# facebookresearch/pytorch3d

Hardware: AMD Instinct MI355X
Metric: rasterized Mpix/s (fwd+bwd) at 512^2 faces_per_pixel=8 (higher is better)
Workload: dtype f32

## Files before the change

pytorch3d_amd/csrc/p3d_geom.h:

```cpp
#pragma once

#include <math.h>
#include <stdint.h>

#if defined(__HIPCC__)
#define P3D_HD __host__ __device__ __forceinline__
#define P3D_HDM __host__ __device__ __forceinline__
#else
#define P3D_HD static inline
#define P3D_HDM inline
#endif

namespace p3d {

#define P3D_KEPS 1e-8

struct f2 {
  float x, y;
};
struct f3 {
  float x, y, z;
};

P3D_HD f2 mk2(float x, float y) {
// ... 179 lines not shown
  f3 v0, v1, v2;
  double rd_area;
  double rd_l01, rd_l02, rd_l12;
  bool wide;
  f2 d01, d12, d20;
};

P3D_HD float edge_fn_d(f2 p, f2 a, f2 d) { return (p.x - a.x) * d.y - (p.y - a.y) * d.x; }

P3D_HD double edge_recip(f2 a, f2 b) {
  const float bax = b.x - a.x;
  const float bay = b.y - a.y;
  const float l2 = bax * bax + bay * bay;
  return ((double)l2 <= P3D_KEPS) ? -1.0 : recip_for_div_wide(l2);
}

P3D_HD void face_rec_make(f3 v0, f3 v1, f3 v2, FaceRec* r) {
  const f2 a = mk2(v0.x, v0.y), b = mk2(v1.x, v1.y), c = mk2(v2.x, v2.y);
  const float area = bary_area(a, b, c);
  r->v0 = v0;
  r->v1 = v1;
  r->v2 = v2;
  r->rd_area = recip_for_div_wide(area);
  r->rd_l01 = edge_recip(a, b);
  r->rd_l02 = edge_recip(a, c);
  r->rd_l12 = edge_recip(b, c);
  r->d01 = mk2(b.x - a.x, b.y - a.y);
  r->d12 = mk2(c.x - b.x, c.y - b.y);
  r->d20 = mk2(a.x - c.x, a.y - c.y);
  const float big = fmaxf(fmaxf(fmaxf(fabsf(v0.x), fabsf(v0.y)), fmaxf(fabsf(v1.x), fabsf(v1.y))),
                          fmaxf(fmaxf(fabsf(v2.x), fabsf(v2.y)), max3(fabsf(v0.z), fabsf(v1.z), fabsf(v2.z))));
  r->wide = !((big <= 1024.0f) & (fabsf(area) >= 1e-9f));
}

template <bool PROPER = false>
P3D_HD float seg_dist2_rec(f2 p, f2 a, f2 b, f2 ba, double rd_l2) {
  const float bax = ba.x;
  const float bay = ba.y;
  float t = exact_div(bax * (p.x - a.x) + bay * (p.y - a.y), rd_l2);
  t = sat01(t);
  const float dx = (a.x + t * bax) - p.x;
  const float dy = (a.y + t * bay) - p.y;
  const float d_seg = dx * dx + dy * dy;
  if (PROPER) return d_seg;
  const float ex = p.x - b.x;
  const float ey = p.y - b.y;
  const float d_point = ex * ex + ey * ey;
  return (rd_l2 < 0.0) ? d_point : d_seg;
}

P3D_HD bool face_rec_degenerate(const FaceRec& r) { return (r.rd_l01 < 0.0) | (r.rd_l02 < 0.0) | (r.rd_l12 < 0.0); }

P3D_HD f3 face_depth_rec(const FaceRec& r, f2 p, bool perspective_correct, bool clip_bary, FaceHit* out) {
  const f2 a = mk2(r.v0.x, r.v0.y);
  const f2 b = mk2(r.v1.x, r.v1.y);
  const f2 c = mk2(r.v2.x, r.v2.y);
  const f3 bw = mk3(exact_div(edge_fn_d(p, b, r.d12), r.rd_area), exact_div(edge_fn_d(p, c, r.d20), r.rd_area),
                    exact_div(edge_fn_d(p, a, r.d01), r.rd_area));
  f3 bp = bw;
  if (perspective_correct) {
    const float t0 = bw.x * r.v1.z * r.v2.z;
    const float t1 = r.v0.z * bw.y * r.v2.z;
    const float t2 = r.v0.z * r.v1.z * bw.z;
    const float denom = fmaxf(t0 + t1 + t2, (float)P3D_KEPS);
    const double rd = r.wide ? recip_for_div_wide(denom) : recip_for_div(denom);
    bp = mk3(exact_div(t0, rd), exact_div(t1, rd), exact_div(t2, rd));
  }
  f3 bc = bp;
  if (clip_bary) {
    const float w0 = bp.x > 0.0f ? bp.x : 0.0f;
    const float w1 = bp.y > 0.0f ? bp.y : 0.0f;
    const float w2 = bp.z > 0.0f ? bp.z : 0.0f;
    float s = w0 + w1 + w2;
    s = fmaxf(s, 1e-5f);
    const double rd = r.wide ? recip_for_div_wide(s) : recip_for_div(s);
    bc = mk3(exact_div(w0, rd), exact_div(w1, rd), exact_div(w2, rd));
  }
  out->z = bc.x * r.v0.z + bc.y * r.v1.z + bc.z * r.v2.z;
  out->bary = bc;
  return bp;
}

template <bool PROPER = false>
P3D_HD bool face_dist_rec(const FaceRec& r, f2 p, float blur_radius, f3 bp, FaceHit* out) {
  const f2 a = mk2(r.v0.x, r.v0.y);
  const f2 b = mk2(r.v1.x, r.v1.y);
  const f2 c = mk2(r.v2.x, r.v2.y);
  const float e01 = seg_dist2_rec<PROPER>(p, a, b, r.d01, r.rd_l01);
  const float e02 = seg_dist2_rec<PROPER>(p, a, c, mk2(-r.d20.x, -r.d20.y), r.rd_l02);
  const float e12 = seg_dist2_rec<PROPER>(p, b, c, r.d12, r.rd_l12);
  const float dist = fminf(fminf(e01, e02), e12);
  const bool inside = (bp.x > 0.0f) & (bp.y > 0.0f) & (bp.z > 0.0f);
  out->dist = inside ? -dist : dist;
  return !(out->z < 0.0f) & (inside | !(dist >= blur_radius));
}

P3D_HD bool face_hit_rec(const FaceRec& r, f2 p, float blur_radius, bool perspective_correct, bool clip_bary,
                         FaceHit* out) {
  const f3 bp = face_depth_rec(r, p, perspective_correct, clip_bary, out);
  return face_dist_rec(r, p, blur_radius, bp, out);
}

P3D_HD unsigned range_mask16(int below, int above) { return (0xffffu >> above) & (0xffffu << below) & 0xffffu; }

P3D_HD void block_mask_8x8(unsigned cols8, unsigned rows8, unsigned* lo, unsigned* hi) {
  *lo = cols8 * (((rows8 & 15u) * 0x00204081u) & 0x01010101u);
  *hi = cols8 * ((((rows8 >> 4) & 15u) * 0x00204081u) & 0x01010101u);
}

P3D_HD bool rect_cannot_hit(f2 a, f2 b, f2 c, float x0, float x1, float y0, float y1, float r) {
  const float big = fmaxf(fmaxf(fmaxf(fabsf(a.x), fabsf(a.y)), fmaxf(fabsf(b.x), fabsf(b.y))), fmaxf(fabsf(c.x), fabsf(c.y)));
  const float rm = r + (2e-5f + 1e-4f * r);
  const float rm2 = rm * rm;
  const float gx = fmaxf(fmaxf(min3(a.x, b.x, c.x) - x1, x0 - max3(a.x, b.x, c.x)), 0.0f);
  const float gy = fmaxf(fmaxf(min3(a.y, b.y, c.y) - y1, y0 - max3(a.y, b.y, c.y)), 0.0f);
  const bool miss_box = gx * gx + gy * gy > rm2;
  bool miss = false;
  const float area = edge_fn(c, a, b);
  const float s = area < 0.0f ? -1.0f : 1.0f;
#define P3D_EDGE_MISS(u, v)                                                                      \
  {                                                                                              \
    const float A = s * (v.y - u.y), B = -s * (v.x - u.x);                                       \
    const float f = A * ((A > 0.0f ? x1 : x0) - u.x) + B * ((B > 0.0f ? y1 : y0) - u.y);         \
    miss = miss | ((f < 0.0f) & (f * f > rm2 * (A * A + B * B)));                                \
  }
  P3D_EDGE_MISS(b, c)
  P3D_EDGE_MISS(c, a)
  P3D_EDGE_MISS(a, b)
#undef P3D_EDGE_MISS
  return (big <= 8.0f) & (miss_box | (miss & (fabsf(area) >= 1e-7f)));
}

struct EdgeGrad {
  f2 dp, da, db;
};

P3D_HD EdgeGrad edge_fn_bwd(f2 p, f2 a, f2 b, float g) {
#if defined(__clang__)
#pragma clang fp contract(fast)
#endif
  EdgeGrad r;
  r.dp = mk2(g * (b.y - a.y), g * (a.x - b.x));
  r.da = mk2(g * (p.y - b.y), g * (b.x - p.x));
  r.db = mk2(g * (a.y - p.y), g * (p.x - a.x));
  return r;
}

struct TriGrad {
  f2 d0, d1, d2;
};

P3D_HD f2 add2(f2 a, f2 b) { return mk2(a.x + b.x, a.y + b.y); }

P3D_HD TriGrad bary_coords_bwd(f2 p, f2 v0, f2 v1, f2 v2, f3 g, f3 e, float inv_area, float inv_area2) {
#if defined(__clang__)
#pragma clang fp contract(fast)
#endif
  const float e0 = e.x, e1 = e.y, e2 = e.z;

  const EdgeGrad n0 = edge_fn_bwd(p, v1, v2, g.x * inv_area);
  const EdgeGrad n1 = edge_fn_bwd(p, v2, v0, g.y * inv_area);
  const EdgeGrad n2 = edge_fn_bwd(p, v0, v1, g.z * inv_area);
  const EdgeGrad ar = edge_fn_bwd(v2, v0, v1, -(g.x * e0 + g.y * e1 + g.z * e2) * inv_area2);

  TriGrad r;
  r.d0 = add2(add2(n1.db, n2.da), ar.da);
  r.d1 = add2(add2(n0.da, n2.db), ar.db);
  r.d2 = add2(add2(n0.db, n1.da), ar.dp);
  return r;
}

P3D_HD f3 bary_clip_bwd(f3 b, f3 g) {
#if defined(__clang__)
#pragma clang fp contract(fast)
#endif
  const float w0 = b.x > 0.0f ? b.x : 0.0f;
  const float w1 = b.y > 0.0f ? b.y : 0.0f;
  const float w2 = b.z > 0.0f ? b.z : 0.0f;
  float s = w0 + w1 + w2;
  float live = 1.0f;
  if ((double)s < 1e-5) {
    live = 0.0f;
    s = 1e-5f;
  }
  const float m0 = b.x < 0.0f ? 0.0f : 1.0f;
  const float m1 = b.y < 0.0f ? 0.0f : 1.0f;
  const float m2 = b.z < 0.0f ? 0.0f : 1.0f;
  const float inv = qdiv<true>(1.0f, s);
  const float inv_s2 = inv * inv * live;
  const float q0 = -w0 * inv_s2;
  const float q1 = -w1 * inv_s2;
  const float q2 = -w2 * inv_s2;
  const float c0 = live != 0.0f ? (w1 + w2) * inv_s2 : inv;
  const float c1 = live != 0.0f ? (w0 + w2) * inv_s2 : inv;
  const float c2 = live != 0.0f ? (w0 + w1) * inv_s2 : inv;
  return mk3(m0 * (g.x * c0 + g.y * q1 + g.z * q2), m1 * (g.y * c1 + g.x * q0 + g.z * q2), m2 * (g.z * c2 + g.x * q0 + g.y * q1));
}

struct FaceGrad {
  float g[9];
};

struct BwdFacePre {
  float inv_area, inv_l01, inv_l02, inv_l12;
};

P3D_HD BwdFacePre bwd_face_pre_make(f3 v0, f3 v1, f3 v2) {
  const f2 a = mk2(v0.x, v0.y), b = mk2(v1.x, v1.y), c = mk2(v2.x, v2.y);
  BwdFacePre r;
  r.inv_area = qdiv<true>(1.0f, bary_area(a, b, c));
  const f2 es[3] = {a, a, b}, ee[3] = {b, c, c};
  float inv[3];
  for (int i = 0; i < 3; ++i) {
    const float bax = ee[i].x - es[i].x, bay = ee[i].y - es[i].y;
    const float l2 = bax * bax + bay * bay;
    inv[i] = (l2 <= 1e-8f) ? -1.0f : qdiv<true>(1.0f, l2);
  }
  r.inv_l01 = inv[0];
  r.inv_l02 = inv[1];
  r.inv_l12 = inv[2];
  return r;
}

template <bool PRE = false>
P3D_HD FaceGrad face_sample_bwd(f3 v0, f3 v1, f3 v2, f2 p, float g_zbuf, f3 g_bary, float g_dist,
                                bool perspective_correct, bool clip_bary, bool clip_bwd_on_corrected,
                                BwdFacePre pre = BwdFacePre()) {
#if defined(__clang__)
#pragma clang fp contract(fast)
#endif
  const f2 a = mk2(v0.x, v0.y);
  const f2 b = mk2(v1.x, v1.y);
  const f2 c = mk2(v2.x, v2.y);
  const float z0 = v0.z, z1 = v1.z, z2 = v2.z;
  const f3 e = mk3(edge_fn(p, b, c), edge_fn(p, c, a), edge_fn(p, a, b));
  float inv_area, inv_area2;
  if (PRE) {
    inv_area = pre.inv_area;
    inv_area2 = inv_area * inv_area;
  } else {
    const float area = bary_area(a, b, c);
    inv_area = qdiv<true>(1.0f, area);
    inv_area2 = qdiv<true>(1.0f, area * area);
  }
  const f3 bw = mk3(e.x * inv_area, e.y * inv_area, e.z * inv_area);
  f3 bp = bw;
  float t0 = 0.0f, t1 = 0.0f, t2 = 0.0f, inv_denom = 0.0f;
  if (perspective_correct) {
    t0 = bw.x * z1 * z2;
    t1 = z0 * bw.y * z2;
    t2 = z0 * z1 * bw.z;
    const float denom = fmaxf(t0 + t1 + t2, (float)P3D_KEPS);
    inv_denom = qdiv<true>(1.0f, denom);
    bp = mk3(t0 * inv_denom, t1 * inv_denom, t2 * inv_denom);
  }
  const f3 bc = clip_bary ? bary_clip<true>(bp) : bp;
  const bool inside = (bp.x > 0.0f) & (bp.y > 0.0f) & (bp.z > 0.0f);
  const float gd = inside ? -g_dist : g_dist;

  float et[3], ex[3], ey[3], ed[3];
  const f2 es[3] = {a, a, b}, ee[3] = {b, c, c};
#pragma unroll
  for (int i = 0; i < 3; ++i) {
    const float bax = ee[i].x - es[i].x, bay = ee[i].y - es[i].y;
    const float dot = bax * (p.x - es[i].x) + bay * (p.y - es[i].y);
    float t;
    bool degenerate;
    if (PRE) {
      const float inv = i == 0 ? pre.inv_l01 : (i == 1 ? pre.inv_l02 : pre.inv_l12);
      degenerate = inv < 0.0f;
      t = sat01(dot * inv);
    } else {
      const float l2 = bax * bax + bay * bay;
      degenerate = l2 <= 1e-8f;
      t = sat01(qdiv<true>(dot, l2));
    }
    const float qx = (es[i].x + t * bax) - p.x, qy = (es[i].y + t * bay) - p.y;
    const float px = p.x - ee[i].x, py = p.y - ee[i].y;
    et[i] = t;
    ex[i] = qx;
    ey[i] = qy;
    ed[i] = degenerate ? px * px + py * py : qx * qx + qy * qy;
  }
  const int sel = ((ed[0] <= ed[1]) & (ed[0] <= ed[2])) ? 0 : (((ed[1] <= ed[0]) & (ed[1] <= ed[2])) ? 1 : (((ed[2] <= ed[0]) & (ed[2] <= ed[1])) ? 2 : 3));
  const float st = sel == 0 ? et[0] : (sel == 1 ? et[1] : et[2]);
  const float sx = sel == 0 ? ex[0] : (sel == 1 ? ex[1] : ex[2]);
  const float sy = sel == 0 ? ey[0] : (sel == 1 ? ey[1] : ey[2]);
  const float g2 = sel == 3 ? 0.0f : gd + gd;
  const float ga = g2 * (1.0f - st), gb_ = g2 * st;
  const f2 da = mk2(ga * sx, ga * sy), db = mk2(gb_ * sx, gb_ * sy);
  const f2 zero = mk2(0.0f, 0.0f);
  const f2 dd0 = sel <= 1 ? da : zero;
  const f2 dd1 = sel == 0 ? db : (sel == 2 ? da : zero);
  const f2 dd2 = (sel == 1 || sel == 2) ? db : zero;

  f3 gb = mk3(g_bary.x + g_zbuf * z0, g_bary.y + g_zbuf * z1, g_bary.z + g_zbuf * z2);
  if (clip_bary) gb = bary_clip_bwd(clip_bwd_on_corrected ? bp : bw, gb);
  float dz0 = 0.0f, dz1 = 0.0f, dz2 = 0.0f;
  if (perspective_correct) {
    const float gd_top = -t0 * gb.x - t1 * gb.y - t2 * gb.z;
    const float gdn = gd_top * (inv_denom * inv_denom);
    const float g0 = gdn + gb.x * inv_denom;
    const float g1 = gdn + gb.y * inv_denom;
    const float g2p = gdn + gb.z * inv_denom;
    dz0 = g1 * bw.y * z2 + g2p * bw.z * z1;
    dz1 = g0 * bw.x * z2 + g2p * bw.z * z0;
    dz2 = g0 * bw.x * z1 + g1 * bw.y * z0;
    gb = mk3(g0 * z1 * z2, g1 * z0 * z2, g2p * z0 * z1);
  }
  const TriGrad dbw = bary_coords_bwd(p, a, b, c, gb, e, inv_area, inv_area2);

  FaceGrad r;
  r.g[0] = dbw.d0.x + dd0.x;
  r.g[1] = dbw.d0.y + dd0.y;
  r.g[2] = g_zbuf * bc.x + dz0;
  r.g[3] = dbw.d1.x + dd1.x;
  r.g[4] = dbw.d1.y + dd1.y;
  r.g[5] = g_zbuf * bc.y + dz1;
  r.g[6] = dbw.d2.x + dd2.x;
  r.g[7] = dbw.d2.y + dd2.y;
  r.g[8] = g_zbuf * bc.z + dz2;
  return r;
}


}
```

pytorch3d_amd/csrc/raster_mesh.hip:

```cpp
#include "binning.h"
#include "tile_map.h"
#include "chunk_order.h"
#include "p3d_geom.h"
#include "topk.h"

#include <stdio.h>
#include <stdlib.h>


#ifdef P3D_PROBE_CHAIN
__device__ unsigned long long g_chain[32];
extern "C" __attribute__((visibility("default"))) void p3d_probe_chain_read(unsigned long long* out) {
  (void)hipDeviceSynchronize();
  (void)hipMemcpyFromSymbol(out, HIP_SYMBOL(g_chain), sizeof(unsigned long long) * 32);
  unsigned long long z[32] = {0};
  (void)hipMemcpyToSymbol(HIP_SYMBOL(g_chain), z, sizeof(z));
}
namespace p3d {
namespace {
constexpr int kChainStamps = 11;
__shared__ unsigned long long s_chain[4][kChainStamps + 1];
__device__ __forceinline__ void chain_note(int i, unsigned long long t) {
  if ((threadIdx.x & 63) == 0) s_chain[threadIdx.x >> 6][i] = t;
}
__device__ __forceinline__ void chain_stamp(int i) { chain_note(i, __builtin_readcyclecounter()); }
__device__ __forceinline__ void chain_flush(unsigned long long r0) {
  const int lane = threadIdx.x & 63, w = threadIdx.x >> 6;
  if (s_chain[w][kChainStamps] == 0ull || lane >= kChainStamps) return;
  if (lane == 0) {
    atomicAdd(&g_chain[15], (unsigned long long)__builtin_amdgcn_s_memrealtime() - r0);
    atomicAdd(&g_chain[31], 1ull);
    return;
  }
  const unsigned long long t1 = s_chain[w][lane];
  int prev = lane - 1;
  while (prev > 0 && s_chain[w][prev] == 0ull) --prev;
  if (t1 == 0ull) return;
  atomicAdd(&g_chain[lane], t1 - s_chain[w][prev]);
  atomicAdd(&g_chain[16 + lane], 1ull);
}
}
}
#define P3D_CHAIN_ENTRY()                                                                                        \
  const unsigned long long chain_t0 = __builtin_readcyclecounter();                                              \
  const unsigned long long chain_r0 = __builtin_amdgcn_s_memrealtime();                                          \
  if ((threadIdx.x & 63) < kChainStamps + 1) s_chain[threadIdx.x >> 6][threadIdx.x & 63] = 0ull
#define P3D_CHAIN_ARM(on)                                                                 \
  if ((on) && (blockIdx.x & 7u) == 0u) {                                                  \
    chain_note(kChainStamps, 1ull);                                                       \
    chain_note(0, chain_t0);                                                              \
  }
#define P3D_CHAIN_STAMP(i) chain_stamp(i)
#define P3D_CHAIN_ARRIVED(i, ...)               \
  do {                                          \
    asm volatile("" ::__VA_ARGS__ : "memory");  \
    chain_stamp(i);                             \
  } while (0)
#define P3D_CHAIN_FLUSH() chain_flush(chain_r0)
#else
#define P3D_CHAIN_ENTRY() ((void)0)
#define P3D_CHAIN_ARM(on) ((void)0)
#define P3D_CHAIN_STAMP(i) ((void)0)
#define P3D_CHAIN_ARRIVED(i, ...) ((void)0)
#define P3D_CHAIN_FLUSH() ((void)0)
#endif

namespace p3d {

namespace {

constexpr int kTile = 16;
constexpr int kStage = 256;
constexpr int kMeshPayload = 4;
constexpr int kSplitMaxTiles = 512;

constexpr int kFineWaves = 4;

struct MeshArgs {
  const float* face_verts;
  const int64_t* neighbor;
  const int64_t* mesh_first;
  const int64_t* mesh_count;
  BinCSR csr;
  int N, H, W, K;
  TileMap tm;
  float blur, sqrt_blur;
  int persp, clip, cull;
  int walk_plan;
  int64_t* p2f;
  float* zbuf;
  float* bary;
  float* dists;
  int* cover;
  int CY, CX;
  int* area_count;
  int* area_list;
  int list_by_plan;
  const int* overflow;
  int ties;
  unsigned long long* tie_words;
  int SY, SX;
};

typedef unsigned int u32x4 __attribute__((ext_vector_type(4)));
__device__ __forceinline__ void store16(void* p, unsigned a, unsigned b, unsigned c, unsigned d) {
  u32x4 v = {a, b, c, d};
  *reinterpret_cast<u32x4*>(p) = v;
}

template <int KT>
__device__ __forceinline__ void store_row(float* dst, const float (&v)[KT]) {
  if constexpr (KT % 4 == 0) {
#pragma unroll
    for (int k = 0; k < KT; k += 4) {
      float4 t;
      t.x = v[k];
      t.y = v[k + 1];
      t.z = v[k + 2];
      t.w = v[k + 3];
      *reinterpret_cast<float4*>(dst + k) = t;
    }
  } else if constexpr (KT == 2) {
    float2 t;
    t.x = v[0];
    t.y = v[1];
    *reinterpret_cast<float2*>(dst) = t;
  } else {
#pragma unroll
    for (int k = 0; k < KT; ++k) dst[k] = v[k];
  }
}

template <typename Queue, int KT, bool IN_REGS>
__device__ __forceinline__ void write_pixel(const MeshArgs& a, const Queue& q, int64_t opix) {
  static_assert(IN_REGS, "vector-row stores need the register queue");
  const int64_t base = opix * KT;
  float zv[KT], dv[KT], bv[3 * KT];
  long long iv[KT];
#pragma unroll
  for (int k = 0; k < KT; ++k) {
    const bool ok = q.valid(k);
    iv[k] = ok ? (long long)q.ix(k) : -1ll;
    zv[k] = ok ? q.zf(k) : -1.0f;
    dv[k] = ok ? q.pay(0, k) : -1.0f;
    bv[3 * k + 0] = ok ? q.pay(1, k) : -1.0f;
    bv[3 * k + 1] = ok ? q.pay(2, k) : -1.0f;
    bv[3 * k + 2] = ok ? q.pay(3, k) : -1.0f;
  }
  if constexpr (KT % 4 == 0) {
#pragma unroll
    for (int k = 0; k < KT; k += 4) {
      store16(a.zbuf + base + k, __float_as_uint(zv[k]), __float_as_uint(zv[k + 1]), __float_as_uint(zv[k + 2]),
                  __float_as_uint(zv[k + 3]));
      store16(a.dists + base + k, __float_as_uint(dv[k]), __float_as_uint(dv[k + 1]), __float_as_uint(dv[k + 2]),
                  __float_as_uint(dv[k + 3]));
    }
#pragma unroll
    for (int k = 0; k < 3 * KT; k += 4)
      store16(a.bary + base * 3 + k, __float_as_uint(bv[k]), __float_as_uint(bv[k + 1]), __float_as_uint(bv[k + 2]),
                  __float_as_uint(bv[k + 3]));
#pragma unroll
// ... 278 lines not shown
        const int jb = __builtin_amdgcn_readlane(oj, cb);
        const float zb = __int_as_float(__builtin_amdgcn_readlane(__float_as_int(zcv), cb));
        jj = mine_is_b ? jb : jj;
        zc = mine_is_b ? zb : zc;
        inside |= in_b;
      }
    }
    const bool in_box = __builtin_amdgcn_inverse_ballot_w64(inside);
    const bool too_deep = zc > q.kth_z(K);
    if (pix_ok && in_box && !too_deep) {
      const float kz0 = TIES ? q.kth_z(K) : 0.0f;
      const int ki0 = TIES ? q.kth_i(K) : 0;
      if constexpr (TIES && GENERAL) tie_z = INFINITY;
      const float4* rec = reinterpret_cast<const float4*>(reinterpret_cast<const char*>(s_rec) + __umul24((unsigned)jj, (unsigned)(kRecWords * sizeof(float4))));
      const float4 r0 = rec[0], r1 = rec[1], r2 = rec[2];
      const int f = __float_as_int(r2.y);
      FaceHit h;
      bool hit = false;
      {
        const double2 d0 = *reinterpret_cast<const double2*>(&rec[3]);
        const double2 d1 = *reinterpret_cast<const double2*>(&rec[4]);
        FaceRec fr;
        fr.v0 = mk3(r0.x, r0.y, r1.z);
        fr.v1 = mk3(r0.z, r0.w, r1.w);
        fr.v2 = mk3(r1.x, r1.y, r2.x);
        fr.rd_area = d0.x;
        fr.rd_l01 = d0.y;
        fr.rd_l02 = d1.x;
        fr.rd_l12 = d1.y;
        const float4 r5 = rec[5];
        const float2 r6 = *reinterpret_cast<const float2*>(&rec[6]);
        fr.d01 = mk2(r5.x, r5.y);
        fr.d12 = mk2(r5.z, r5.w);
        fr.d20 = mk2(r6.x, r6.y);
        const bool pcs = PC && !GENERAL;
        fr.wide = pcs ? false : __float_as_int(r2.w) != 0;
        const f3 bp = face_depth_rec(fr, p, pcs || persp, pcs || clip, &h);
        const bool adm = !(h.z < 0.0f) & q.admits(K, h.z, f);
        if constexpr (TIES && !GENERAL) {
          const bool ev = (h.z == kz0) & !adm;
          const int d = kz0 == tie_z ? min(tie_drop, f) : f;
          tie_drop = ev ? d : tie_drop;
          tie_z = ev ? kz0 : tie_z;
        }
        if (GENERAL || adm) hit = face_dist_rec<PC && !GENERAL>(fr, p, a.blur, bp, &h);
      }
      if (hit) {
        bool ins = true;
        if constexpr (GENERAL) {
          const int nb = __float_as_int(r2.z);
          if (nb != -1) {
            const int at = q.find(nb);
            if (at >= 0) {
              float queued;
              if constexpr (Queue::kPayload > 0) {
                queued = q.payload_at(0, at);
              } else {
                queued = recompute_face(a, nb, p, persp, clip).dist;
              }
              if (fabsf(h.dist) < fabsf(queued))
                q.erase(at);
              else
                ins = false;
            }
          }
        }
        if (ins && q.admits(K, h.z, f)) {
          if constexpr (Queue::kPayload > 0) {
            const float pl[kMeshPayload] = {h.dist, h.bary.x, h.bary.y, h.bary.z};
            q.insert(K, h.z, f, pl);
          } else {
            const float none[1] = {0.0f};
            q.insert(K, h.z, f, none);
          }
          if constexpr (TIES && !GENERAL) {
            const bool ev = (kz0 < INFINITY) & (q.kth_z(K) == kz0);
            const int d = kz0 == tie_z ? min(tie_drop, ki0) : ki0;
            tie_drop = ev ? d : tie_drop;
            tie_z = ev ? kz0 : tie_z;
          }
        }
      }
    }
  }
}

__device__ __forceinline__ void cover_mark(const MeshArgs& a, int n, int sy0, bool any, int yo, int xo, int lane) {
  unsigned long long rem = __ballot(any);
  const int wid = (yo >> 4) * a.CX + (xo >> 4);
  while (rem) {
    const int w0 = __builtin_amdgcn_readlane(wid, __builtin_ctzll(rem));
    const unsigned long long same = __ballot(any && wid == w0);
    unsigned bits = 0;
#pragma unroll
    for (int j = 0; j < 8; ++j)
      if ((same >> (8 * j)) & 0xffull) bits |= 1u << ((a.H - 1 - (sy0 + j)) & 15);
    rem &= ~same;
    if (lane == 0) {
      const int word = (n * a.CY) * a.CX + w0;
      if (a.area_list != nullptr && !a.list_by_plan) {
        const int before = atomicOr(a.cover + word, (int)bits);
        if (before == 0 && bits != 0u) a.area_list[atomicAdd(a.area_count, 1)] = word;
      } else {
        atomicOr(a.cover + word, (int)bits);
      }
    }
  }
}

__device__ __forceinline__ float uniform_f(float v) { return __int_as_float(__builtin_amdgcn_readfirstlane(__float_as_int(v))); }

struct StageLds {
  unsigned* pm;
  float pxy;
  unsigned valid_c, valid_r;
  float4 (*rec)[kRecWords];
  float* zc;
  int* order;
  float* qlow;
  ChunkOrderScratch* ord;
  int* wcnt;
};

struct TileRect {
  float x0, x1, y0, y1;
};

template <bool BINNED, bool PC = false>
__device__ __forceinline__ int stage_chunk(const MeshArgs& a, const StageLds& l, const TileRect& tile, int64_t src_base,
                                           int count, int base, int tid, bool cull, bool clip, bool prune, bool* general) {
  const int lane = tid & 63, w = tid >> 6;
  const int i = base + tid;
  bool keep = false;
  f3 v0, v1, v2;
  FaceSetup fs;
  int fid = -1, nb = -1;
  unsigned cm = 0, rm = 0;
  const bool has = i < count;
  fs.xlo = fs.xhi = fs.ylo = fs.yhi = 0.0f;
  fs.reject = true;
  if (has) {
    fid = BINNED ? a.csr.list[src_base + i] : (int)(src_base + i);
    P3D_CHAIN_ARRIVED(2, "v"(fid));
    const float* g = a.face_verts + (int64_t)fid * 9;
    nb = (int)a.neighbor[fid];
    v0 = mk3(g[0], g[1], g[2]);
    v1 = mk3(g[3], g[4], g[5]);
    v2 = mk3(g[6], g[7], g[8]);
    P3D_CHAIN_ARRIVED(3, "v"(v0.x), "v"(v1.y), "v"(v2.z), "v"(nb));
    fs = face_setup(v0, v1, v2, a.sqrt_blur, cull);
  }
  int xb = 0, xa = 0, yb = 0, ya = 0;
  if (__ballot(has) != 0) {
#pragma unroll
    for (int c = 0; c < 16; ++c) {
      const float xs = __int_as_float(__builtin_amdgcn_readlane(__float_as_int(l.pxy), c));
      const float ys = __int_as_float(__builtin_amdgcn_readlane(__float_as_int(l.pxy), 16 + c));
      xb += xs < fs.xlo ? 1 : 0;
      xa += xs > fs.xhi ? 1 : 0;
      yb += ys < fs.ylo ? 1 : 0;
      ya += ys > fs.yhi ? 1 : 0;
    }
  }
  if (has) {
    cm = range_mask16(xb, xa) & l.valid_c;
    rm = range_mask16(yb, ya) & l.valid_r;
    keep = !fs.reject && cm != 0 && rm != 0;
    if (keep && prune)
      keep = !rect_cannot_hit(mk2(v0.x, v0.y), mk2(v1.x, v1.y), mk2(v2.x, v2.y), tile.x0, tile.x1, tile.y0, tile.y1, a.sqrt_blur);
  }
  const unsigned long long km = __ballot(keep);
  if (lane == 0) l.wcnt[w] = __popcll(km);
  __syncthreads();
  int pos = mask_rank(km);
  int staged = 0;
#pragma unroll
  for (int j = 0; j < kStage / kWave; ++j) {
    const int c = l.wcnt[j];
    if (j < w) pos += c;
    staged += c;
  }
  bool gen = false;
  if (keep) {
    FaceRec fr;
    face_rec_make(v0, v1, v2, &fr);
    gen = nb != -1 || (PC && (fr.wide || face_rec_degenerate(fr)));
    l.pm[pos] = cm | (rm << 16);
    l.rec[pos][0] = make_float4(v0.x, v0.y, v1.x, v1.y);
    l.rec[pos][1] = make_float4(v2.x, v2.y, v0.z, v1.z);
    l.rec[pos][2] = make_float4(v2.z, __int_as_float(fid), __int_as_float(nb), __int_as_float(fr.wide ? 1 : 0));
    double2 d0, d1;
    d0.x = fr.rd_area;
    d0.y = fr.rd_l01;
    d1.x = fr.rd_l02;
    d1.y = fr.rd_l12;
    *reinterpret_cast<double2*>(&l.rec[pos][3]) = d0;
    *reinterpret_cast<double2*>(&l.rec[pos][4]) = d1;
    l.rec[pos][5] = make_float4(fr.d01.x, fr.d01.y, fr.d12.x, fr.d12.y);
    l.rec[pos][6] = make_float4(fr.d20.x, fr.d20.y, 0.0f, 0.0f);
    const float zmin = min3(v0.z, v1.z, v2.z);
    l.zc[pos] = (clip && nb == -1 && zmin >= 1e-3f) ? zmin * 0.999998f : -INFINITY;
  }
  *general = __syncthreads_or(gen ? 1 : 0) != 0;
  return staged;
}

struct SubTile {
  float x0, x1, y0, y1;
};

template <bool GENERAL, typename Queue, bool PC = false, bool TIES = false>
__device__ __forceinline__ void wave_chunk(const MeshArgs& a, int K, Queue& q, int staged, bool sorted, const SubTile& st, f2 p,
                                           bool pix_ok, int lane, bool persp, bool clip, bool prune, const unsigned* s_pm,
                                           const float4 (*s_rec)[kRecWords], const float* s_zc, const int* s_order,
                                           const float* s_qlow, int cshift, int rshift, float& tie_z, int& tie_drop, int deal = -1) {
  for (int jb = 0; jb < staged; jb += kWave) {
    const int jfirst = deal >= 0 ? deal * 16 : jb;
    if (jfirst >= staged) break;
    if (sorted && __ballot(pix_ok && !(s_qlow[jfirst] > q.kth_z(K))) == 0) break;
    const int j = deal >= 0 ? (((lane >> 4) * 4 + deal) * 16 + (lane & 15)) : jb + lane;
    bool touch = false;
    int oj = 0;
    unsigned mlo = 0, mhi = 0;
    float zcv = 0.0f;
    if (j < staged) {
      oj = s_order[j];
      const unsigned pm = s_pm[oj];
      const unsigned cmask = (pm >> cshift) & 0xffu, rmask = (pm >> (16 + rshift)) & 0xffu;
      touch = (cmask != 0) & (rmask != 0);
      if (touch && prune) {
        const float4 r0 = s_rec[oj][0], r1 = s_rec[oj][1];
        touch = !rect_cannot_hit(mk2(r0.x, r0.y), mk2(r0.z, r0.w), mk2(r1.x, r1.y), st.x0, st.x1, st.y0, st.y1, a.sqrt_blur);
      }
      block_mask_8x8(cmask, rmask, &mlo, &mhi);
      zcv = s_zc[oj];
    }
    const unsigned long long cand = __ballot(touch);
    eval_candidates<GENERAL, Queue, PC, TIES>(a, K, q, cand, oj, mlo, mhi, zcv, p, pix_ok, persp, clip, s_rec, tie_z, tie_drop);
    if (deal >= 0) break;
  }
}

constexpr int kMergeWords = 2 + kMeshPayload;

template <typename Queue, int KT>
__device__ __forceinline__ void merge_dump(const Queue& q, float* slab, int lane) {
#pragma unroll
  for (int k = 0; k < KT; ++k) {
    slab[(0 * KT + k) * kWave + lane] = q.zf(k);
    slab[(1 * KT + k) * kWave + lane] = __int_as_float(q.ix(k));
#pragma unroll
    for (int pp = 0; pp < kMeshPayload; ++pp) slab[((2 + pp) * KT + k) * kWave + lane] = q.pay(pp, k);
  }
}

template <typename Queue, int KT>
__device__ __forceinline__ void merge_absorb(Queue& q, int K, const float* slab, int lane) {
#pragma unroll 1
  for (int k = 0; k < KT; ++k) {
    const int idx = __float_as_int(slab[(1 * KT + k) * kWave + lane]);
    if (__ballot(idx != kEmptyIdx) == 0) break;
    const float z = slab[(0 * KT + k) * kWave + lane];
    float pl[kMeshPayload];
#pragma unroll
    for (int pp = 0; pp < kMeshPayload; ++pp) pl[pp] = slab[((2 + pp) * KT + k) * kWave + lane];
    if (idx != kEmptyIdx && q.admits(K, z, idx)) q.insert(K, z, idx, pl);
  }
}

template <typename Queue, int KT, bool IN_REGS, bool BINNED, bool EXACT, int WAVES = kFineWaves, bool PC = false,
          bool SPLIT = false, bool TIES = false>
__global__ __launch_bounds__(kStage, WAVES) void mesh_raster_kernel(MeshArgs a) {
  static_assert(!(SPLIT && TIES), "the tie marks of four queues that merge are not tracked: CUDA tie order runs the plain kernels");
  __shared__ float s_merge[SPLIT ? 3 * kMergeWords * KT * kWave : 1];
  __shared__ unsigned s_pm[kStage];
  __shared__ float4 s_rec[kStage][kRecWords];
  __shared__ __align__(16) float s_zc[kStage];
  __shared__ int s_order[kStage];
  __shared__ float s_qlow[kStage];
  __shared__ ChunkOrderScratch s_ord;
  __shared__ int s_wcnt[kStage / kWave];
  __shared__ int s_fill_ticket;

  P3D_CHAIN_ENTRY();
  __builtin_amdgcn_s_setprio(3);
  unsigned blk = SPLIT ? blockIdx.x >> 2 : blockIdx.x;
  const bool plan_walk = BINNED && !SPLIT && a.walk_plan != 0;
  int hdr_a = 0, hdr_b = 0, hdr_order = 0;
  int walk_row = 0;
  if (plan_walk) {
    hdr_a = a.csr.plan.hdr[0];
    hdr_b = a.csr.plan.hdr[1];
    hdr_order = a.csr.plan.hdr[3];
    const unsigned rows = (unsigned)(a.N * a.tm.BH * a.tm.BW);
    walk_row = a.csr.plan.order[blk < rows ? blk : rows - 1u];
  }
  if (a.overflow != nullptr && (*a.overflow != 0) == BINNED) return;
  TileCoord tc;
  bool listed = false;
  if (plan_walk && hdr_order != 0) {
    const unsigned A = (unsigned)hdr_a, B = (unsigned)hdr_b;
    int row;
    if (blk < A) {
      row = walk_row;
    } else if (blk < A + B) {
      if (EXACT && (KT & 3) == 0 && A > 0) return;
      row = a.csr.plan.bg_list[blk - A];
    } else {
      return;
    }
    const int per_image = a.tm.BH * a.tm.BW;
    tc.n = row / per_image;
    const int rem = row - tc.n * per_image;
    tc.by = rem / a.tm.BW;
    tc.bx = rem - tc.by * a.tm.BW;
    tc.ty = tc.tx = 0;
    if (blk < A && a.list_by_plan && threadIdx.x == 0) {
      a.area_list[blk] = (tc.n * a.CY + (a.CY - 1 - tc.by)) * a.CX + (a.CX - 1 - tc.bx);
      if (blk == 0) *a.area_count = (int)A;
    }
    listed = true;
  }
  if (!listed && !tile_of_block(a.tm, blk, &tc)) return;
  const int n = tc.n, by = tc.by, bx = tc.bx, ty = tc.ty, tx = tc.tx;

  const int H = a.H, W = a.W;
  const int y_end = min(H, (by + 1) * a.tm.bin_size);
  const int x_end = min(W, (bx + 1) * a.tm.bin_size);
  const int ty0 = by * a.tm.bin_size + ty * kTile;
  const int tx0 = bx * a.tm.bin_size + tx * kTile;
  if (ty0 >= y_end || tx0 >= x_end) return;

  const int tid = threadIdx.x;
  const int lane = tid & 63;
  const int w = __builtin_amdgcn_readfirstlane(tid >> 6);
  const int sub = SPLIT ? (int)(blockIdx.x & 3u) : w;
  const int sy0 = ty0 + (sub >> 1) * 8;
  const int sx0 = tx0 + (sub & 1) * 8;
  if (SPLIT && (sy0 >= y_end || sx0 >= x_end)) return;
  const int yi = sy0 + (lane >> 3);
  const int xi = sx0 + (lane & 7);
  const bool pix_ok = yi < y_end && xi < x_end;
  const bool wave_ok = sy0 < y_end && sx0 < x_end;

  const bool piggy = BINNED && !SPLIT && EXACT && (KT & 3) == 0 && plan_walk;
  int64_t src_base;
  int count;
  int fill_slot = (int)blk;
  if (BINNED) {
    const int64_t row = ((int64_t)n * a.tm.BH + by) * a.tm.BW + bx;
    count = a.csr.total[row];
    src_base = a.csr.offset[row];
    if (!listed && (piggy || (!SPLIT && a.list_by_plan))) fill_slot = a.csr.plan.arank[row];
  } else {
// ... 778 lines not shown
```

pytorch3d_amd/csrc/raster_mesh_bwd.hip:

```cpp
#include "p3d_common.h"
#include "p3d_geom.h"
#include "wave_table.h"

#include <stdlib.h>

#include <type_traits>

namespace p3d {

namespace {

constexpr int kRegion = 32;
constexpr int kBwdSlots = 182;
using FaceTable = WaveTable<9, kBwdSlots, kRows>;
using FaceTableV = WaveTable<9, kBwdSlots, kCorners>;

struct BwdArgs {
  const float* face_verts;
  const int64_t* p2f;
  const float* grad_zbuf;
  const float* grad_bary;
  const float* grad_dists;
  float* grad_fv;
  const int64_t* faces;
// ... 257 lines not shown
#endif

template <int KT, bool PRE = false>
struct RowsCfg {
  static constexpr bool kSeven = PRE && KT <= 8;
  static constexpr int kWaves = KT >= 16 ? 5 : (kSeven ? P3D_BWD_WAVES : 6);
  static constexpr int kQueue = KT <= 8 ? (kSeven ? P3D_BWD_QUEUE : P3D_BWD_QUEUE6) : 0;
  static constexpr bool kPacked = KT <= 8 && P3D_BWD_PACKED;
  static constexpr int kSlots = KT >= 16 ? 136 : (kSeven ? P3D_BWD_SLOTS : P3D_BWD_SLOTS6);
  static constexpr int kPix = 64 / KT;
};

template <int CTRL>
__device__ __forceinline__ int dpp_i(int v) {
  return __builtin_amdgcn_update_dpp(0, v, CTRL, 0xf, 0xf, true);
}
template <int CTRL>
__device__ __forceinline__ float dpp_f(float v) {
  return __int_as_float(__builtin_amdgcn_update_dpp(0, __float_as_int(v), CTRL, 0xf, 0xf, true));
}

template <int D, int PIX>
__device__ __forceinline__ void run_level(bool e, float (&g)[9]) {
  if constexpr (D < PIX) {
#pragma unroll
    for (int j = 0; j < 9; ++j) {
      const float sum = g[j] + dpp_f<0x110 + D>(g[j]);
      g[j] = e ? sum : g[j];
    }
  }
}

template <int PIX>
__device__ __forceinline__ void run_reduce(int& f, float (&g)[9], int lane) {
  const int pix = lane & (PIX - 1);
  const int f_left = dpp_i<0x111>(f);
  const int f_right = dpp_i<0x101>(f);
  const int e1 = (pix >= 1) & (f >= 0) & (f_left == f);
  const int e1_left = dpp_i<0x111>(e1);
  const int e2 = PIX > 2 ? (e1 & e1_left) : 0;
  const int e2_left = dpp_i<0x112>(e2);
  const int e4 = PIX > 4 ? (e2 & e2_left) : 0;
  const int e4_left = dpp_i<0x114>(e4);
  const int e8 = PIX > 8 ? (e4 & e4_left) : 0;
  const bool continues = (pix < PIX - 1) & (f_right == f);
  run_level<1, PIX>(e1 != 0, g);
  run_level<2, PIX>(e2 != 0, g);
  run_level<4, PIX>(e4 != 0, g);
  run_level<8, PIX>(e8 != 0, g);
  if (continues) f = -1;
}

template <int KT, bool TO_VERTS, bool PC = false, bool PRE = false>
__global__ __launch_bounds__(256, (RowsCfg<KT, PRE>::kWaves)) void mesh_backward_rows_kernel(BwdArgs a) {
  constexpr int SPR = KT / 4;
  constexpr int PIX = RowsCfg<KT>::kPix;
  static_assert(KT == 4 || KT == 8 || KT == 16 || KT == 32, "16 K samples per row segment, 64 per step");
  using Cfg = RowsCfg<KT, PRE>;
  using Table = WaveTable<9, Cfg::kSlots, TO_VERTS ? kCorners : kRows, true, true, Cfg::kPacked>;
  constexpr int QCAP = Cfg::kQueue;
  static_assert(Table::kLdsInts % 4 == 0, "every wave's table starts on a 16-byte boundary");
  __shared__ __align__(16) int s_table[4][Table::kLdsInts + 10 * QCAP];
  static_assert((sizeof(s_table) + 1279) / 1280 * 1280 * Cfg::kWaves <= 160 * 1024, "kWaves workgroups do not fit the CU's LDS (1280-byte pieces)");

  const int tid = threadIdx.x;
  const int lane = tid & 63;
  const int w = __builtin_amdgcn_readfirstlane(tid >> 6);
  const unsigned item = blockIdx.x * 4u + (unsigned)w;
  unsigned area;
  if (a.area_list != nullptr) {
    if (item >= (unsigned)*a.area_count) return;
    area = (unsigned)a.area_list[item];
  } else {
    if (item >= a.nblocks) return;
    area = (unsigned)(((unsigned long long)item * a.scatter) % a.nblocks);
  }
  const int cx = (int)(area % (unsigned)a.CX);
  const unsigned t = area / (unsigned)a.CX;
  const int cy = (int)(t % (unsigned)a.CY);
  const int n = (int)(t / (unsigned)a.CY);
  const int ay = cy * 16, ax = cx * 16;
  const int H = a.H, W = a.W;
  const int rows = min(16, H - ay);
  unsigned todo = area_rows(a, n, ay, ax) & ((1u << rows) - 1u);
  if (todo == 0) return;

  Table tab;
  tab.init(s_table[w], lane);
  tab.index = a.faces;
  tab.index_limit = a.V;
  const bool persp = PC || a.persp != 0, clip = PC || a.clip != 0;

  const int seg = min(16, W - ax) * KT;
  const int e = (lane & (PIX - 1)) * KT + lane / PIX;
  float px[SPR];
#pragma unroll
  for (int s = 0; s < SPR; ++s) {
    px[s] = pix_to_ndc(W - 1 - (ax + s * PIX + (lane & (PIX - 1))), W, H);
    asm volatile("" : "+v"(px[s]));
  }
  float py_rows = pix_to_ndc(H - 1 - (ay + (lane & 15)), H, W);
  asm volatile("" : "+v"(py_rows));
  const int64_t area_base = (((int64_t)n * H + ay) * W + ax) * KT;
  const int64_t row_pitch = (int64_t)W * KT;

  const unsigned eu = (unsigned)e, eu3 = 3u * (unsigned)e;
  int rn = __builtin_ctz(todo), sn = 0;
  todo &= todo - 1;
  int f_nxt = e < seg ? (int)uniform_ptr(a.p2f + (area_base + (int64_t)rn * row_pitch))[eu] : -1;
  typedef __attribute__((address_space(3))) int LdsQInt;
  typedef __attribute__((address_space(3))) float LdsQFloat;
  [[maybe_unused]] LdsQInt* const q_f = (LdsQInt*)(s_table[w] + Table::kLdsInts);
  [[maybe_unused]] LdsQFloat* const q_g = (LdsQFloat*)(s_table[w] + Table::kLdsInts + QCAP);
  [[maybe_unused]] int cnt = 0;
#pragma unroll 1
  while (rn >= 0 || (QCAP > 0 && cnt > 0)) {
    const bool tail = QCAP > 0 && rn < 0;
    int f = -1;
    FaceGrad g;
    if (!tail) {
      const int r = rn, s = sn;
      f = f_nxt;
      if (++sn == SPR) {
        sn = 0;
        rn = todo ? __builtin_ctz(todo) : -1;
        todo &= todo - 1;
      }
      {
        const int en = 64 * sn + e;
        const auto* prow = uniform_ptr(a.p2f + (area_base + (int64_t)(rn < 0 ? 0 : rn) * row_pitch + 64 * sn));
        f_nxt = (rn >= 0 && en < seg) ? (int)prow[eu] : -1;
      }
      if (__ballot(f >= 0) == 0) continue;
      if (f >= 0) {
        const int64_t rb = area_base + (int64_t)r * row_pitch + 64 * s;
        const auto* gzp = uniform_ptr(a.grad_zbuf + rb);
        const auto* gdp = uniform_ptr(a.grad_dists + rb);
        const auto* gbp = uniform_ptr(a.grad_bary + 3 * rb);
        const float gz = gzp[eu], gd = gdp[eu];
        const f3 gb = mk3(gbp[eu3], gbp[eu3 + 1u], gbp[eu3 + 2u]);
        const float* q = a.face_verts + (int64_t)f * 9;
        float pxs = px[0];
#pragma unroll
        for (int c = 1; c < SPR; ++c) pxs = s == c ? px[c] : pxs;
        const f2 p = mk2(pxs, __int_as_float(__builtin_amdgcn_readlane(__float_as_int(py_rows), r)));
        BwdFacePre pre = BwdFacePre();
        if constexpr (PRE) {
          const float4 r = a.face_pre[f];
          pre.inv_area = r.x;
          pre.inv_l01 = r.y;
          pre.inv_l02 = r.z;
          pre.inv_l12 = r.w;
        }
        g = face_sample_bwd<PRE>(mk3(q[0], q[1], q[2]), mk3(q[3], q[4], q[5]), mk3(q[6], q[7], q[8]), p, gz, gb, gd, persp, clip, false, pre);
      } else {
#pragma unroll
        for (int j = 0; j < 9; ++j) g.g[j] = 0.0f;
      }
      run_reduce<PIX>(f, g.g, lane);
    } else {
#pragma unroll
      for (int j = 0; j < 9; ++j) g.g[j] = 0.0f;
    }
    if constexpr (QCAP > 0) {
      const unsigned long long m = __ballot(f >= 0);
      const int S = __popcll(m);
      if (!tail && cnt + S <= QCAP) {
        if (f >= 0) {
          const int i = cnt + mask_rank(m);
          q_f[i] = f;
#pragma unroll
          for (int j = 0; j < 9; ++j) q_g[j * QCAP + i] = g.g[j];
        }
        __builtin_amdgcn_fence(__ATOMIC_RELEASE, "wavefront");
        cnt += S;
        continue;
      }
      const int take = min(cnt, 64 - S);
      __builtin_amdgcn_fence(__ATOMIC_ACQUIRE, "wavefront");
      if (f < 0) {
        const int rk = mask_rank(~m);
        if (rk < take) {
          const int i = cnt - 1 - rk;
          f = q_f[i];
#pragma unroll
          for (int j = 0; j < 9; ++j) g.g[j] = q_g[j * QCAP + i];
        }
      }
      __builtin_amdgcn_fence(__ATOMIC_ACQ_REL, "wavefront");
      cnt -= take;
    }
    tab.add(a.grad_fv, lane, f, g.g);
  }
  if (tab.used > 0) tab.flush(a.grad_fv, lane);
}

}

}

using namespace p3d;

P3D_API size_t p3d_rasterize_meshes_backward_workspace_bytes(int N, int H, int W);

namespace {
int launch_mesh_backward(const float* face_verts, const int64_t* faces, int64_t V, const int64_t* p2f, const float* grad_zbuf,
                         const float* grad_bary, const float* grad_dists, int N, int H, int W, int K, int persp, int clip,
                         float* grad_out, const int32_t* cover, void* workspace, size_t workspace_bytes, hipStream_t s,
                         bool cover_has_list, const float* face_pre) {
  BwdArgs a;
  a.face_pre = reinterpret_cast<const float4*>(face_pre);
  a.V = V;
  a.face_verts = face_verts;
  a.p2f = p2f;
  a.grad_zbuf = grad_zbuf;
  a.grad_bary = grad_bary;
  a.grad_dists = grad_dists;
  a.grad_fv = grad_out;
  a.faces = faces;
  a.N = N;
  a.H = H;
  a.W = W;
  a.K = K;
  a.RY = (int)ceil_div(H, kRegion);
  a.RX = (int)ceil_div(W, kRegion);
  a.persp = persp;
  a.clip = clip;
  a.cover = cover;
  a.CY = (H + 15) / 16;
  a.CX = (W + 15) / 16;
  a.area_list = nullptr;
  a.area_count = nullptr;
  const bool rows_kernel = K == 4 || K == 8 || K == 16 || K == 32;
  const int64_t items = rows_kernel ? (int64_t)N * a.CY * a.CX : (int64_t)N * a.RY * a.RX;
  if (items > 0x7fffffffll) return P3D_ERR_INVALID_ARG;
  a.nblocks = (unsigned)items;
  a.scatter = scatter_multiplier((uint64_t)items);
  if (rows_kernel && cover != nullptr && cover_has_list) {
    const int* count = reinterpret_cast<const int*>(cover) + items;
    a.area_list = count + 16;
    a.area_count = count;
  } else if (rows_kernel && cover != nullptr && workspace != nullptr &&
      workspace_bytes >= p3d_rasterize_meshes_backward_workspace_bytes(N, H, W)) {
    int* count = static_cast<int*>(workspace);
    int* list = count + 16;
    if (hipMemsetAsync(count, 0, sizeof(int), s) != hipSuccess) return P3D_ERR_LAUNCH;
    LaunchScope ls("mesh_backward_areas", s);
    area_list_kernel<<<(unsigned)ceil_div(items, 256), 256, 0, s>>>(cover, (int)items, list, count);
    a.area_list = list;
    a.area_count = count;
  }
  LaunchScope ls("mesh_backward", s);
  const unsigned grid = rows_kernel ? (unsigned)ceil_div(items, 4) : (unsigned)items;
  const bool pc = persp && clip;
#define P3D_LAUNCH_MESH_BWD(TV)                                                  \
  switch (K) {                                                                   \
    case 1: mesh_backward_kernel<1, TV><<<grid, 256, 0, s>>>(a); break;          \
    case 2: mesh_backward_kernel<2, TV><<<grid, 256, 0, s>>>(a); break;          \
    case 4:                                                                      \
      if (pc && a.face_pre) mesh_backward_rows_kernel<4, TV, true, true><<<grid, 256, 0, s>>>(a); \
      else if (pc) mesh_backward_rows_kernel<4, TV, true><<<grid, 256, 0, s>>>(a); \
      else mesh_backward_rows_kernel<4, TV><<<grid, 256, 0, s>>>(a);             \
      break;                                                                     \
    case 8:                                                                      \
      if (pc && a.face_pre) mesh_backward_rows_kernel<8, TV, true, true><<<grid, 256, 0, s>>>(a); \
      else if (pc) mesh_backward_rows_kernel<8, TV, true><<<grid, 256, 0, s>>>(a); \
      else mesh_backward_rows_kernel<8, TV><<<grid, 256, 0, s>>>(a);             \
      break;                                                                     \
    case 16: mesh_backward_rows_kernel<16, TV><<<grid, 256, 0, s>>>(a); break;   \
    case 32: mesh_backward_rows_kernel<32, TV><<<grid, 256, 0, s>>>(a); break;   \
    default: mesh_backward_kernel<0, TV><<<grid, 256, 0, s>>>(a); break;         \
  }
  if (faces) {
    P3D_LAUNCH_MESH_BWD(true)
  } else {
    P3D_LAUNCH_MESH_BWD(false)
  }
#undef P3D_LAUNCH_MESH_BWD
  return launch_status();
}
}

P3D_API size_t p3d_rasterize_meshes_backward_workspace_bytes(int N, int H, int W) {
  if (N <= 0 || H <= 0 || W <= 0) return 0;
  return ((size_t)N * (size_t)((H + 15) / 16) * (size_t)((W + 15) / 16) + 16) * sizeof(int);
}

P3D_API int p3d_rasterize_meshes_backward_ex(const float* face_verts, const int64_t* faces, float* face_pre, const int64_t* p2f,
                                              const float* grad_zbuf, const float* grad_bary, const float* grad_dists, const int32_t* cover,
                                              int64_t F, int64_t V, int N, int H, int W, int K, int persp, int clip, unsigned flags,
                                              float* grad_out, void* workspace, size_t workspace_bytes, p3d_stream_t stream) {
  if (F < 0 || V < 0 || N < 0 || H < 0 || W < 0 || K < 0) return P3D_ERR_INVALID_ARG;
  if ((flags & ~(P3D_BWD_COVER_HAS_LIST | P3D_BWD_MAKE_FACE_PRE)) != 0 || ((uintptr_t)face_pre & 15u)) return P3D_ERR_INVALID_ARG;
  const int64_t out_floats = faces ? V * 3 : F * 9;
  if (out_floats == 0) return P3D_OK;
  if (!grad_out) return P3D_ERR_INVALID_ARG;
  hipStream_t s = (hipStream_t)stream;
  if (hipMemsetAsync(grad_out, 0, (size_t)out_floats * sizeof(float), s) != hipSuccess) return P3D_ERR_LAUNCH;
  if (F == 0 || (int64_t)N * H * W * K == 0) return P3D_OK;
  if (!face_verts || !p2f || !grad_zbuf || !grad_bary || !grad_dists) return P3D_ERR_INVALID_ARG;
  if (flags & P3D_BWD_MAKE_FACE_PRE) {
    if (face_pre != nullptr && persp && clip && (K == 4 || K == 8)) {
      int64_t blocks = ceil_div(F, 256);
      if (blocks > 256 * 16) blocks = 256 * 16;
      LaunchScope ls("face_pre", s);
      face_pre_kernel<<<(unsigned)blocks, 256, 0, s>>>(face_verts, F, reinterpret_cast<float4*>(face_pre));
      const int st = launch_status();
// ... 34 lines not shown
```

Before: 7940.

## Pack backward face-gradient math into float2 FMAs and index staging ranges arithmetically

The backward per-face gradient code gets a packed float2 FMA variant, covering the barycentric backward, clip backward, segment projection and final assembly. It is enabled only for the precomputed, perspective-correct queued configuration, so the compiler can emit packed FMA instructions on MI355X. Separately, forward staging replaces a 16-iteration readlane loop that counts pixel columns and rows outside a face's range with a direct index estimate from reciprocal spacing plus two bpermute corrections. A NaN guard is also added to the z-cull value, and the estimate assumes evenly spaced pixel centres.

```diff
diff --git a/pytorch3d_amd/csrc/p3d_geom.h b/pytorch3d_amd/csrc/p3d_geom.h
--- a/pytorch3d_amd/csrc/p3d_geom.h
+++ b/pytorch3d_amd/csrc/p3d_geom.h
@@ -355,6 +355,35 @@
 
 P3D_HD f2 add2(f2 a, f2 b) { return mk2(a.x + b.x, a.y + b.y); }
 
+#ifndef P3D_BWD_PK
+#define P3D_BWD_PK 1
+#endif
+#if defined(__HIP_DEVICE_COMPILE__) && P3D_BWD_PK
+typedef float pk2 __attribute__((ext_vector_type(2)));
+P3D_HD pk2 pk_mk(float x, float y) {
+  pk2 r = {x, y};
+  return r;
+}
+P3D_HD pk2 pk_fma(pk2 a, pk2 b, pk2 c) { return __builtin_elementwise_fma(a, b, c); }
+#else
+struct pk2 {
+  float x, y;
+};
+P3D_HD pk2 pk_mk(float x, float y) {
+  pk2 r;
+  r.x = x;
+  r.y = y;
+  return r;
+}
+P3D_HD pk2 pk_fma(pk2 a, pk2 b, pk2 c) {
+#if defined(__clang__)
+#pragma clang fp contract(fast)
+#endif
+  return pk_mk(a.x * b.x + c.x, a.y * b.y + c.y);
+}
+#endif
+P3D_HD pk2 pk_all(float s) { return pk_mk(s, s); }
+
 P3D_HD TriGrad bary_coords_bwd(f2 p, f2 v0, f2 v1, f2 v2, f3 g, f3 e, float inv_area, float inv_area2) {
 #if defined(__clang__)
 #pragma clang fp contract(fast)
@@ -373,6 +402,26 @@
   return r;
 }
 
+P3D_HD TriGrad bary_coords_bwd_pk(f2 p, f2 v0, f2 v1, f2 v2, f3 g, f3 e, float inv_area, float inv_area2) {
+#if defined(__clang__)
+#pragma clang fp contract(fast)
+#endif
+  const float G0 = g.x * inv_area, G1 = g.y * inv_area, G2 = g.z * inv_area;
+  const float GA = -(g.x * e.x + g.y * e.y + g.z * e.z) * inv_area2;
+  const pk2 P0 = pk_mk(p.y - v0.y, v0.x - p.x), P1 = pk_mk(p.y - v1.y, v1.x - p.x), P2 = pk_mk(p.y - v2.y, v2.x - p.x);
+  const pk2 E01 = pk_mk(v1.y - v0.y, v0.x - v1.x), E12 = pk_mk(v2.y - v1.y, v1.x - v2.x), E20 = pk_mk(v0.y - v2.y, v2.x - v0.x);
+  const float nG0 = -G0, nG1 = -G1, nG2 = -G2;
+  const pk2 d0 = pk_fma(pk_all(GA), E12, pk_fma(pk_all(G2), P1, pk_mk(nG1 * P2.x, nG1 * P2.y)));
+  const pk2 d1 = pk_fma(pk_all(GA), E20, pk_fma(pk_all(nG2), P0, pk_mk(G0 * P2.x, G0 * P2.y)));
+  const pk2 d2 = pk_fma(pk_all(GA), E01, pk_fma(pk_all(G1), P0, pk_mk(nG0 * P1.x, nG0 * P1.y)));
+  TriGrad r;
+  r.d0 = mk2(d0.x, d0.y);
+  r.d1 = mk2(d1.x, d1.y);
+  r.d2 = mk2(d2.x, d2.y);
+  return r;
+}
+
+template <bool PK = false>
 P3D_HD f3 bary_clip_bwd(f3 b, f3 g) {
 #if defined(__clang__)
 #pragma clang fp contract(fast)
@@ -397,6 +446,10 @@
   const float c0 = live != 0.0f ? (w1 + w2) * inv_s2 : inv;
   const float c1 = live != 0.0f ? (w0 + w2) * inv_s2 : inv;
   const float c2 = live != 0.0f ? (w0 + w1) * inv_s2 : inv;
+  if (PK) {
+    const pk2 s01 = pk_fma(pk_all(g.z), pk_all(q2), pk_fma(pk_mk(g.y, g.x), pk_mk(q1, q0), pk_mk(g.x * c0, g.y * c1)));
+    return mk3(m0 * s01.x, m1 * s01.y, m2 * (g.z * c2 + g.x * q0 + g.y * q1));
+  }
   return mk3(m0 * (g.x * c0 + g.y * q1 + g.z * q2), m1 * (g.y * c1 + g.x * q0 + g.z * q2), m2 * (g.z * c2 + g.x * q0 + g.y * q1));
 }
 
@@ -425,7 +478,7 @@
   return r;
 }
 
-template <bool PRE = false>
+template <bool PRE = false, bool PK = false>
 P3D_HD FaceGrad face_sample_bwd(f3 v0, f3 v1, f3 v2, f2 p, float g_zbuf, f3 g_bary, float g_dist,
                                 bool perspective_correct, bool clip_bary, bool clip_bwd_on_corrected,
                                 BwdFacePre pre = BwdFacePre()) {
@@ -478,7 +531,15 @@
       degenerate = l2 <= 1e-8f;
       t = sat01(qdiv<true>(dot, l2));
     }
-    const float qx = (es[i].x + t * bax) - p.x, qy = (es[i].y + t * bay) - p.y;
+    float qx, qy;
+    if (PK) {
+      const pk2 c = pk_fma(pk_all(t), pk_mk(bax, bay), pk_mk(es[i].x, es[i].y));
+      qx = c.x - p.x;
+      qy = c.y - p.y;
+    } else {
+      qx = (es[i].x + t * bax) - p.x;
+      qy = (es[i].y + t * bay) - p.y;
+    }
     const float px = p.x - ee[i].x, py = p.y - ee[i].y;
     et[i] = t;
     ex[i] = qx;
@@ -498,22 +559,49 @@
   const f2 dd2 = (sel == 1 || sel == 2) ? db : zero;
 
   f3 gb = mk3(g_bary.x + g_zbuf * z0, g_bary.y + g_zbuf * z1, g_bary.z + g_zbuf * z2);
-  if (clip_bary) gb = bary_clip_bwd(clip_bwd_on_corrected ? bp : bw, gb);
+  if (clip_bary) gb = bary_clip_bwd<PK>(clip_bwd_on_corrected ? bp : bw, gb);
   float dz0 = 0.0f, dz1 = 0.0f, dz2 = 0.0f;
   if (perspective_correct) {
     const float gd_top = -t0 * gb.x - t1 * gb.y - t2 * gb.z;
     const float gdn = gd_top * (inv_denom * inv_denom);
-    const float g0 = gdn + gb.x * inv_denom;
-    const float g1 = gdn + gb.y * inv_denom;
+    float g0, g1;
+    if (PK) {
+      const pk2 g01 = pk_fma(pk_mk(gb.x, gb.y), pk_all(inv_denom), pk_all(gdn));
+      g0 = g01.x;
+      g1 = g01.y;
+    } else {
+      g0 = gdn + gb.x * inv_denom;
+      g1 = gdn + gb.y * inv_denom;
+    }
     const float g2p = gdn + gb.z * inv_denom;
     dz0 = g1 * bw.y * z2 + g2p * bw.z * z1;
     dz1 = g0 * bw.x * z2 + g2p * bw.z * z0;
     dz2 = g0 * bw.x * z1 + g1 * bw.y * z0;
     gb = mk3(g0 * z1 * z2, g1 * z0 * z2, g2p * z0 * z1);
   }
-  const TriGrad dbw = bary_coords_bwd(p, a, b, c, gb, e, inv_area, inv_area2);
+  const TriGrad dbw = PK ? bary_coords_bwd_pk(p, a, b, c, gb, e, inv_area, inv_area2) : bary_coords_bwd(p, a, b, c, gb, e, inv_area, inv_area2);
 
   FaceGrad r;
+  if (PK) {
+    const float w0 = sel <= 1 ? ga : 0.0f;
+    const float w1 = sel == 0 ? gb_ : (sel == 2 ? ga : 0.0f);
+    const float w2 = (sel == 1 || sel == 2) ? gb_ : 0.0f;
+    const pk2 sxy = pk_mk(sx, sy);
+    const pk2 r0 = pk_fma(pk_all(w0), sxy, pk_mk(dbw.d0.x, dbw.d0.y));
+    const pk2 r1 = pk_fma(pk_all(w1), sxy, pk_mk(dbw.d1.x, dbw.d1.y));
+    const pk2 r2 = pk_fma(pk_all(w2), sxy, pk_mk(dbw.d2.x, dbw.d2.y));
+    const pk2 z01 = pk_fma(pk_all(g_zbuf), pk_mk(bc.x, bc.y), pk_mk(dz0, dz1));
+    r.g[0] = r0.x;
+    r.g[1] = r0.y;
+    r.g[2] = z01.x;
+    r.g[3] = r1.x;
+    r.g[4] = r1.y;
+    r.g[5] = z01.y;
+    r.g[6] = r2.x;
+    r.g[7] = r2.y;
+    r.g[8] = g_zbuf * bc.z + dz2;
+    return r;
+  }
   r.g[0] = dbw.d0.x + dd0.x;
   r.g[1] = dbw.d0.y + dd0.y;
   r.g[2] = g_zbuf * bc.x + dz0;
diff --git a/pytorch3d_amd/csrc/raster_mesh.hip b/pytorch3d_amd/csrc/raster_mesh.hip
--- a/pytorch3d_amd/csrc/raster_mesh.hip
+++ b/pytorch3d_amd/csrc/raster_mesh.hip
@@ -7,6 +7,9 @@
 #include <stdio.h>
 #include <stdlib.h>
 
+#ifndef P3D_STAGE_RANGE_INDEX
+#define P3D_STAGE_RANGE_INDEX 1
+#endif
 
 #ifdef P3D_PROBE_CHAIN
 __device__ unsigned long long g_chain[32];
@@ -591,6 +594,29 @@
   }
   int xb = 0, xa = 0, yb = 0, ya = 0;
   if (__ballot(has) != 0) {
+#if P3D_STAGE_RANGE_INDEX
+    float pxy = l.pxy;
+    asm volatile("" : "+v"(pxy));
+    const float x0 = __int_as_float(__builtin_amdgcn_readlane(__float_as_int(pxy), 0));
+    const float y0 = __int_as_float(__builtin_amdgcn_readlane(__float_as_int(pxy), 16));
+    const float inv_dx = 15.0f * __builtin_amdgcn_rcpf(__int_as_float(__builtin_amdgcn_readlane(__float_as_int(pxy), 15)) - x0);
+    const float inv_dy = 15.0f * __builtin_amdgcn_rcpf(__int_as_float(__builtin_amdgcn_readlane(__float_as_int(pxy), 31)) - y0);
+    const int rxl = (int)rintf(fminf(fmaxf((fs.xlo - x0) * inv_dx, 0.0f), 15.0f));
+    const int rxh = (int)rintf(fmaxf(fminf((fs.xhi - x0) * inv_dx, 15.0f), 0.0f));
+    const float cxl = __int_as_float(__builtin_amdgcn_ds_bpermute(rxl << 2, __float_as_int(pxy)));
+    const float cxh = __int_as_float(__builtin_amdgcn_ds_bpermute(rxh << 2, __float_as_int(pxy)));
+    xb = rxl + (cxl < fs.xlo ? 1 : 0);
+    xa = 15 - rxh + (cxh > fs.xhi ? 1 : 0);
+    cm = range_mask16(xb, xa) & l.valid_c;
+    __builtin_amdgcn_sched_barrier(0);
+    const int ryl = (int)rintf(fminf(fmaxf((fs.ylo - y0) * inv_dy, 0.0f), 15.0f));
+    const int ryh = (int)rintf(fmaxf(fminf((fs.yhi - y0) * inv_dy, 15.0f), 0.0f));
+    const float cyl = __int_as_float(__builtin_amdgcn_ds_bpermute((16 + ryl) << 2, __float_as_int(pxy)));
+    const float cyh = __int_as_float(__builtin_amdgcn_ds_bpermute((16 + ryh) << 2, __float_as_int(pxy)));
+    yb = ryl + (cyl < fs.ylo ? 1 : 0);
+    ya = 15 - ryh + (cyh > fs.yhi ? 1 : 0);
+    rm = range_mask16(yb, ya) & l.valid_r;
+#else
 #pragma unroll
     for (int c = 0; c < 16; ++c) {
       const float xs = __int_as_float(__builtin_amdgcn_readlane(__float_as_int(l.pxy), c));
@@ -600,10 +626,11 @@
       yb += ys < fs.ylo ? 1 : 0;
       ya += ys > fs.yhi ? 1 : 0;
     }
-  }
-  if (has) {
     cm = range_mask16(xb, xa) & l.valid_c;
     rm = range_mask16(yb, ya) & l.valid_r;
+#endif
+  }
+  if (has) {
     keep = !fs.reject && cm != 0 && rm != 0;
     if (keep && prune)
       keep = !rect_cannot_hit(mk2(v0.x, v0.y), mk2(v1.x, v1.y), mk2(v2.x, v2.y), tile.x0, tile.x1, tile.y0, tile.y1, a.sqrt_blur);
@@ -638,7 +665,7 @@
     l.rec[pos][5] = make_float4(fr.d01.x, fr.d01.y, fr.d12.x, fr.d12.y);
     l.rec[pos][6] = make_float4(fr.d20.x, fr.d20.y, 0.0f, 0.0f);
     const float zmin = min3(v0.z, v1.z, v2.z);
-    l.zc[pos] = (clip && nb == -1 && zmin >= 1e-3f) ? zmin * 0.999998f : -INFINITY;
+    l.zc[pos] = (clip && nb == -1 && zmin >= 1e-3f && fr.rd_area == fr.rd_area) ? zmin * 0.999998f : -INFINITY;
   }
   *general = __syncthreads_or(gen ? 1 : 0) != 0;
   return staged;
diff --git a/pytorch3d_amd/csrc/raster_mesh_bwd.hip b/pytorch3d_amd/csrc/raster_mesh_bwd.hip
--- a/pytorch3d_amd/csrc/raster_mesh_bwd.hip
+++ b/pytorch3d_amd/csrc/raster_mesh_bwd.hip
@@ -433,7 +433,7 @@
           pre.inv_l02 = r.z;
           pre.inv_l12 = r.w;
         }
-        g = face_sample_bwd<PRE>(mk3(q[0], q[1], q[2]), mk3(q[3], q[4], q[5]), mk3(q[6], q[7], q[8]), p, gz, gb, gd, persp, clip, false, pre);
+        g = face_sample_bwd<PRE, P3D_BWD_PK && PRE && PC && (RowsCfg<KT, PRE>::kQueue > 0)>(mk3(q[0], q[1], q[2]), mk3(q[3], q[4], q[5]), mk3(q[6], q[7], q[8]), p, gz, gb, gd, persp, clip, false, pre);
       } else {
 #pragma unroll
         for (int j = 0; j < 9; ++j) g.g[j] = 0.0f;
```

After: 8100 (median of 6 runs). 1.02x the previous value.
